# mpsops/mps-bitsandbytes

Measured on AMD Instinct MI355X. Metric: effective bf16 TFLOPS, NF4 dequant+matmul 4096x4096 @ M=4096 (dequantise-once + dense GEMM, two launches), higher is better.
Workload: dtype bf16

## Files before the change

mps_bitsandbytes_amd/csrc/gemm_dense.h:

```cpp
#pragma once
#include "gemm256.h"
#include <type_traits>
#include <utility>

namespace mbnb {

template <int... I, class F> __device__ __forceinline__ void gd_static_for_impl(std::integer_sequence<int, I...>, F &&f) {
    (f(std::integral_constant<int, I>{}), ...);
}
template <int N, class F> __device__ __forceinline__ void gd_static_for(F &&f) {
    gd_static_for_impl(std::make_integer_sequence<int, N>{}, static_cast<F &&>(f));
}

constexpr int GD_LDS = 4 * P_IMG;

template <int FM, int FN = 8> struct GdPlan {
    static_assert(FN == 8 || (FM == 8 && FN >= 5 && FN <= 7), "narrow tiles exist for the 256-row tile only");
    static constexpr int NS = 2 * FN * FM, NR = FN + FM, NP = FN + FM;
    static constexpr int RS1 = (FM == 8 && FN >= 7) ? 2 : 1;
    static constexpr int B1 = FM != 8 ? 16 : (FN == 8 ? 36 : FN == 7 ? 32 : FN == 6 ? 16 : 13), D0 = B1;
    static constexpr int DS = FM == 8 ? 4 : 2;
    static constexpr int B2 = FM != 8 ? 42 : (FN == 8 ? 100 : FN == 7 ? 94 : FN == 6 ? 78 : 66), R0 = B2;
    static_assert(R0 >= FN * FM, "the next tile's slice 0 replaces this tile's only after its MFMAs");
    static_assert((NR - 1) * RS1 < B1, "slice 1 is in registers before barrier 1");
    static_assert(D0 + NP * DS <= B2, "every piece is issued before the vmcnt of barrier 2");
    static_assert(R0 + NR <= NS, "the next tile's slice 0 is in registers before the k-step ends");
};

__device__ __forceinline__ int gd_xcd_major(int bid, int nwg) {
    const int full = (nwg >> 8) << 8;
    if (bid < full) {
        const int i = bid >> 3;
        return (((i >> 5) << 3) + (bid & 7)) * 32 + (i & 31);
    }
    const int rest = nwg - full, r = bid - full, q = rest >> 3, rr = rest & 7, xcd = r & 7;
    return full + (xcd < rr ? xcd * (q + 1) : rr * (q + 1) + (xcd - rr) * q) + (r >> 3);
}
template <int PM, int PN> __device__ __forceinline__ void gd_patch_walk(int v, int tiles_m, int tiles_n, int &tm, int &tn) {
    const int col_tiles = tiles_m * PN, pcs = tiles_n / PN, prs = tiles_m / PM;
    int pc = v / col_tiles, w = PN;
    if (pc >= pcs) { pc = pcs; w = tiles_n - pcs * PN; }
    const int v1 = v - pc * col_tiles;
    int pr = v1 / (PM * w), h = PM;
    if (pr >= prs) { pr = prs; h = tiles_m - prs * PM; }
    const int v2 = v1 - pr * PM * w;
    tm = pr * PM + v2 % h;
    tn = pc * PN + v2 / h;
}

template <typename T, bool SPLITK, int FM, bool I8, int OUTL, int NCH, int FN>
__device__ __forceinline__ void gemm_dense_body(const T *__restrict__ X, const T *__restrict__ Wd, const T *__restrict__ bias,
                                                void *__restrict__ out_v, int out_dtype, float *__restrict__ partial,
                                                int64_t M, int64_t N, int64_t K, int64_t ldw, int64_t k_per_slice,
                                                const float *__restrict__ sA, const float *__restrict__ sB, const OutlierEpilogue &ep,
                                                const int64_t m0, const int64_t n0, const int slice) {
    static_assert(!(I8 && SPLITK), "the int8 form is not split");
    static_assert(OUTL == 0 || I8, "the outlier epilogue belongs to the int8 form");
    static_assert(OUTL == 0 || FN == 8, "the outlier epilogue is written for the 256-wide tile");
    using Frag = typename Mfma16<T>::frag;
    using Plan = GdPlan<FM, FN>;
    constexpr int TM = 32 * FM, TN = 32 * FN;
    extern __shared__ __attribute__((aligned(1024))) char smem[];
    const int tid = threadIdx.x;
    const int lane = tid & 63;
    const int wave = __builtin_amdgcn_readfirstlane(tid >> 6);
    const int wn = wave >> 1, wm = wave & 1;
    const int64_t k_begin = SPLITK ? (int64_t)slice * k_per_slice : 0;
    const int64_t k_len = SPLITK ? (K - k_begin < k_per_slice ? K - k_begin : k_per_slice) : K;
    const int nk = (int)(k_len >> 6);

    typedef int i32x4_t __attribute__((ext_vector_type(4)));
    i32x4_t rs_a, rs_b;
    {
        const uint64_t pa = reinterpret_cast<uint64_t>(X + m0 * K + k_begin), pb = reinterpret_cast<uint64_t>(Wd + n0 * ldw + k_begin);
        const int64_t rows_a = M - m0 < TM ? M - m0 : TM, rows_b = N - n0 < TN ? N - n0 : TN;
        rs_a = i32x4_t{(int)(uint32_t)pa, (int)(uint32_t)(pa >> 32), (int)(rows_a * K * 2), 0x00020000};
        rs_b = i32x4_t{(int)(uint32_t)pb, (int)(uint32_t)(pb >> 32), (int)(rows_b * ldw * 2), 0x00020000};
    }
    int voff_a[FM], voff_b[FN];
#pragma unroll
    for (int pl = 0; pl < FN; pl++) {
        const int row = 8 * (FN * wave + pl) + (lane >> 3);
        voff_b[pl] = (int)(row * ldw * 2) + 16 * ((lane & 7) ^ ((row >> 1) & 7));
    }
#pragma unroll
    for (int pl = 0; pl < FM; pl++) {
        const int row = 8 * (FM * wave + pl) + (lane >> 3);
        voff_a[pl] = (int)(row * K * 2) + 16 * ((lane & 7) ^ ((row >> 1) & 7));
    }
#pragma unroll
    for (int pl = 0; pl < FN; pl++) voff_b[pl] -= (pl & 3) * 1024;
#pragma unroll
    for (int pl = 0; pl < FM; pl++) voff_a[pl] -= (pl & 3) * 1024;
    const uint32_t smem_base = (uint32_t)(uintptr_t)(__attribute__((address_space(3))) void *)smem;
    struct DmaCtx { i32x4_t ra, rb; uint32_t lwa, lwb; };
    auto dma_ctx = [&]() {
        DmaCtx c;
#pragma unroll
        for (int e = 0; e < 4; e++) {
            c.ra[e] = __builtin_amdgcn_readfirstlane(rs_a[e]);
            c.rb[e] = __builtin_amdgcn_readfirstlane(rs_b[e]);
        }
        c.lwa = (uint32_t)__builtin_amdgcn_readfirstlane((int)(smem_base + (uint32_t)(P_A + wave * FM * 1024)));
        c.lwb = (uint32_t)__builtin_amdgcn_readfirstlane((int)(smem_base + (uint32_t)(P_B + wave * FN * 1024)));
        return c;
    };
    auto issue_piece = [&](auto qq, int stage, int kb, const DmaCtx &c) {
        constexpr int q = decltype(qq)::value, pl = q < FM ? q : q - FM;
        const uint32_t dst = (q < FM ? c.lwa : c.lwb) + (uint32_t)(stage * P_IMG + pl * 1024);
        const int vo = (q < FM) ? voff_a[pl] : voff_b[pl];
        const i32x4_t rs = (q < FM) ? c.ra : c.rb;
        if constexpr ((pl & 3) != 0) {
            asm volatile("buffer_load_dwordx4 %0, %1, %2 offen offset:%3 lds" ::"v"(vo), "s"(rs), "s"(kb), "n"((pl & 3) * 1024) : "memory", "m0");
        } else {
            asm volatile("s_mov_b32 m0, %0\n\ts_nop 0\n\tbuffer_load_dwordx4 %1, %2, %3 offen lds" ::"s"(dst), "v"(vo), "s"(rs), "s"(kb) : "memory", "m0");
        }
    };

    const int r16 = lane & 15, fq = lane >> 4;
    int fw[2], fx[2];
#pragma unroll
    for (int ks = 0; ks < 2; ks++) {
        const int f = r16 * ROW_BYTES + (((4 * ks + fq) ^ (r16 >> 1)) << 4);
        fw[ks] = P_B + wn * 16 * FN * ROW_BYTES + f;
        fx[ks] = P_A + wm * 16 * FM * ROW_BYTES + f;
    }
    Frag wf[2][FN], xf[2][FM];
    auto read_one = [&](int stage, auto kk, auto nn) {
        constexpr int ks = decltype(kk)::value, n = decltype(nn)::value;
        if constexpr (n == 0) wf[ks][0] = *reinterpret_cast<const Frag *>(smem + fw[ks] + stage * P_IMG);
        else if constexpr (n <= FM) xf[ks][n - 1] = *reinterpret_cast<const Frag *>(smem + fx[ks] + stage * P_IMG + (n - 1) * 16 * ROW_BYTES);
        else wf[ks][n - FM] = *reinterpret_cast<const Frag *>(smem + fw[ks] + stage * P_IMG + (n - FM) * 16 * ROW_BYTES);
    };
    f32x4 acc[FN][FM];

    auto kbytes = [&](int t) { return t << 7; };

    {
        const DmaCtx c0 = dma_ctx();
        gd_static_for<Plan::NP>([&](auto q) { issue_piece(q, 0, 0, c0); });
        if (nk > 1) {
            gd_static_for<Plan::NP>([&](auto q) { issue_piece(q, 1, kbytes(1), c0); });
            asm volatile("s_waitcnt vmcnt(%0)" ::"n"(Plan::NP) : "memory");
        } else {
            asm volatile("s_waitcnt vmcnt(0)" ::: "memory");
        }
    }
    __builtin_amdgcn_s_barrier();
    asm volatile("" ::: "memory");
    gd_static_for<Plan::NR>([&](auto n) { read_one(0, std::integral_constant<int, 0>{}, n); });

    auto mfma_acc = [&](f32x4 &c, const Frag &a, const Frag &b) {
        if constexpr (I8) asm volatile("v_mfma_i32_16x16x64_i8 %0, %1, %2, %0" : "+a"(c) : "v"(a), "v"(b));
        else if constexpr (std::is_same_v<T, bf16_t>) asm volatile("v_mfma_f32_16x16x32_bf16 %0, %1, %2, %0" : "+a"(c) : "v"(a), "v"(b));
        else asm volatile("v_mfma_f32_16x16x32_f16 %0, %1, %2, %0" : "+a"(c) : "v"(a), "v"(b));
    };
    auto mfma_zero = [&](f32x4 &c, const Frag &a, const Frag &b) {
        if constexpr (I8) asm volatile("v_mfma_i32_16x16x64_i8 %0, %1, %2, 0" : "=a"(c) : "v"(a), "v"(b));
        else if constexpr (std::is_same_v<T, bf16_t>) asm volatile("v_mfma_f32_16x16x32_bf16 %0, %1, %2, 0" : "=a"(c) : "v"(a), "v"(b));
        else asm volatile("v_mfma_f32_16x16x32_f16 %0, %1, %2, 0" : "=a"(c) : "v"(a), "v"(b));
    };

    auto kstep = [&](auto cc, auto first, auto mode_, auto wo_, int j, const DmaCtx &dc) {
        constexpr int WO = decltype(wo_)::value, MODE = decltype(mode_)::value;
        constexpr bool FIRST = decltype(first)::value;
        const int C = cc, Nn = C ^ 1;
        int kb2 = 0;
        if constexpr (MODE == 0) kb2 = __builtin_amdgcn_readfirstlane(kbytes(j + 2));
        gd_static_for<Plan::NS>([&](auto tt) {
            constexpr int t = decltype(tt)::value, ks = t / (FN * FM), f = (t % (FN * FM)) / FM, g = t % FM;
            if constexpr (t == Plan::B1 && MODE != 2) {
                asm volatile("s_waitcnt lgkmcnt(0)" ::: "memory");
                __builtin_amdgcn_s_barrier();
                asm volatile("" ::: "memory");
            }
            if constexpr (t == Plan::B2 && MODE != 2) {
                asm volatile("s_waitcnt vmcnt(%0)" ::"n"(MODE == 0 ? Plan::NP : 0) : "memory");
                __builtin_amdgcn_s_barrier();
                asm volatile("" ::: "memory");
            }
            if constexpr (FIRST && ks == 0) mfma_zero(acc[f][g], wf[ks][f], xf[ks][g]);
            else mfma_acc(acc[f][g], wf[ks][f], xf[ks][g]);
            if constexpr ((t % Plan::RS1) == 0 && t / Plan::RS1 < Plan::NR)
                read_one(C, std::integral_constant<int, 1>{}, std::integral_constant<int, (t / Plan::RS1) % Plan::NR>{});
            if constexpr (MODE != 2 && t >= Plan::R0 && t < Plan::R0 + Plan::NR)
                read_one(Nn, std::integral_constant<int, 0>{}, std::integral_constant<int, (t - Plan::R0) % Plan::NR>{});
            if constexpr (MODE == 0 && t >= Plan::D0 && t < Plan::D0 + Plan::NP * Plan::DS && ((t - Plan::D0) % Plan::DS) == WO)
                issue_piece(std::integral_constant<int, ((t - Plan::D0) / Plan::DS) % Plan::NP>{}, C, kb2, dc);
            __builtin_amdgcn_sched_barrier(0);
        });
    };
    using Mode0 = std::integral_constant<int, 0>;
    using Mode1 = std::integral_constant<int, 1>;
    using Mode2 = std::integral_constant<int, 2>;
    auto main_loop = [&](auto wo) {
        if (nk < 3) return;
        const DmaCtx dc = dma_ctx();
        kstep(std::integral_constant<int, 0>{}, std::true_type{}, Mode0{}, wo, 0, dc);
        int j = 1;
        for (; j + 3 < nk; j += 2) {
            kstep(std::integral_constant<int, 1>{}, std::false_type{}, Mode0{}, wo, j, dc);
            kstep(std::integral_constant<int, 0>{}, std::false_type{}, Mode0{}, wo, j + 1, dc);
        }
        if (j + 2 < nk) kstep(std::integral_constant<int, 1>{}, std::false_type{}, Mode0{}, wo, j, dc);
    };
    if constexpr (Plan::DS == 4) {
        if (wave == 0) main_loop(std::integral_constant<int, 0>{});
        else if (wave == 1) main_loop(std::integral_constant<int, 1>{});
        else if (wave == 2) main_loop(std::integral_constant<int, 2>{});
        else main_loop(std::integral_constant<int, 3>{});
    } else {
        if ((wave & 1) == 0) main_loop(std::integral_constant<int, 0>{});
        else main_loop(std::integral_constant<int, 1>{});
    }

    constexpr bool TAIL = !SPLITK && !I8 && OUTL == 0 && FN == 8;
    bool tail_ok = false;
    if constexpr (TAIL)
        tail_ok = nk >= 2 && out_dtype == (std::is_same_v<T, f16_t> ? MBNB_F16 : MBNB_BF16) && (N % 8 == 0) &&
                  ((reinterpret_cast<uintptr_t>(out_v) & 15) == 0) && N < ((int64_t)1 << 23);
    u32x2 bias_t[TAIL ? FN : 1];
    if constexpr (TAIL) {
        if (tail_ok && bias != nullptr) {
            const uint16_t *bp = reinterpret_cast<const uint16_t *>(bias);
#pragma unroll
            for (int f = 0; f < FN; f++) {
                const int64_t n = n0 + wn * 16 * FN + 16 * f + 4 * fq;
                if (n + 4 <= N && (reinterpret_cast<uintptr_t>(bp + n) & 7) == 0) bias_t[f] = *reinterpret_cast<const u32x2 *>(bp + n);
                else {
                    uint32_t t[4];
#pragma unroll
                    for (int e = 0; e < 4; e++) t[e] = bp[n + e < N ? n + e : N - 1];
                    bias_t[f] = u32x2{t[0] | (t[1] << 16), t[2] | (t[3] << 16)};
                }
            }
        }
    }
    {
        const DmaCtx none{};
        if (nk == 2) kstep(std::integral_constant<int, 0>{}, std::true_type{}, Mode1{}, std::integral_constant<int, 0>{}, 0, none);
        else if (nk > 2) kstep(nk & 1, std::false_type{}, Mode1{}, std::integral_constant<int, 0>{}, nk - 2, none);
        if (nk == 1) kstep(std::integral_constant<int, 0>{}, std::true_type{}, Mode2{}, std::integral_constant<int, 0>{}, 0, none);
        else if (!tail_ok) kstep((nk - 1) & 1, std::false_type{}, Mode2{}, std::integral_constant<int, 0>{}, nk - 1, none);
    }
    if constexpr (TAIL) {
        auto tail_step = [&](auto wb_t, const int C) {
            constexpr bool WB = decltype(wb_t)::value;
            constexpr int ROWB = 264, GS = 2 * FN;
            int tid2 = threadIdx.x;
            asm volatile("" : "+v"(tid2));
            const int lane_e = tid2 & 63, er16 = lane_e & 15, efq = lane_e >> 4;
            char *stg = smem + (wn ? P_B : P_A) + (C ^ 1) * P_IMG + wm * (2 * 16 * ROWB);
            char *st_w = stg + er16 * ROWB + 8 * efq;
            const char *st_r = stg + efq * ROWB + er16 * 16;
            const int64_t m_w = m0 + wm * 16 * FM;
            int64_t rows = M - m_w;
            rows = rows < 0 ? 0 : (rows > 16 * FM ? 16 * FM : rows);
            const uint64_t po = reinterpret_cast<uint64_t>(static_cast<uint16_t *>(out_v) + m_w * N);
            i32x4_t rs_o;
            rs_o[0] = __builtin_amdgcn_readfirstlane((int)(uint32_t)po);
            rs_o[1] = __builtin_amdgcn_readfirstlane((int)(uint32_t)(po >> 32));
            rs_o[2] = __builtin_amdgcn_readfirstlane((int)(rows * N * 2));
            rs_o[3] = 0x00020000;
            const int rowstep = __builtin_amdgcn_readfirstlane((int)(N * 2));
            const int64_t n = n0 + wn * 16 * FN + er16 * 8;
            const int voff0 = n < N ? (int)((efq * N + n) * 2) : (int)0x80000000;
            u32x4 piece[4];
            auto filler = [&](auto gg, auto ss) {
                constexpr int g = decltype(gg)::value, s = decltype(ss)::value, buf = (g & 1) * 16 * ROWB;
                if constexpr (s < FN) {
                    float bv[4] = {0.0f, 0.0f, 0.0f, 0.0f};
                    if constexpr (WB) {
#pragma unroll
                        for (int e = 0; e < 4; e++) bv[e] = unpack_lo<T>(bias_t[s][e >> 1] >> (16 * (e & 1)));
                    }
                    float v[4];
#pragma unroll
                    for (int e = 0; e < 4; e++) {
                        float sv;
                        asm volatile("v_accvgpr_read_b32 %0, %1" : "=v"(sv) : "a"(acc[s][g][e]));
                        v[e] = sv + bv[e];
                    }
                    const u32x2 pk = u32x2{pack2<T>(v[0], v[1]), pack2<T>(v[2], v[3])};
                    *reinterpret_cast<u32x2 *>(st_w + buf + 32 * s) = pk;
                } else if constexpr (s < FN + 4) {
                    constexpr int p = s - FN;
                    const char *srcp = st_r + buf + p * 4 * ROWB;
                    const u32x2 lo = *reinterpret_cast<const u32x2 *>(srcp), hi = *reinterpret_cast<const u32x2 *>(srcp + 8);
                    piece[p] = u32x4{lo[0], lo[1], hi[0], hi[1]};
                } else if constexpr (s < FN + 8) {
                    constexpr int p = s - FN - 4;
                    const int vo = voff0 + (16 * g + 4 * p) * rowstep;
                    const i32x4_t rs = rs_o;
                    const u32x4 pv = piece[p];
                    asm volatile("buffer_store_dwordx4 %0, %1, %2, 0 offen sc1\n\ts_nop 1" ::"v"(pv), "v"(vo), "s"(rs) : "memory");
                }
            };
            gd_static_for<Plan::NS>([&](auto tt) {
                constexpr int t = decltype(tt)::value, g = t / GS, ks = (t % GS) / FN, f = t % FN;
                if constexpr (std::is_same_v<T, bf16_t>) asm volatile("s_nop 1\n\tv_mfma_f32_16x16x32_bf16 %0, %1, %2, %0" : "+a"(acc[f][g]) : "v"(wf[ks][f]), "v"(xf[ks][g]));
                else asm volatile("s_nop 1\n\tv_mfma_f32_16x16x32_f16 %0, %1, %2, %0" : "+a"(acc[f][g]) : "v"(wf[ks][f]), "v"(xf[ks][g]));
                if constexpr (t < Plan::NR)
                    read_one(C, std::integral_constant<int, 1>{},
                             std::integral_constant<int, (t == 0 ? 1 : t == 1 ? 0 : t <= FN ? t - 1 + FM : t - FN + 1)>{});
                if constexpr (t >= GS) filler(std::integral_constant<int, t / GS - 1>{}, std::integral_constant<int, t % GS>{});
                __builtin_amdgcn_sched_barrier(0);
            });
            gd_static_for<GS>([&](auto ss) {
                filler(std::integral_constant<int, FM - 1>{}, ss);
                __builtin_amdgcn_sched_barrier(0);
            });
        };
        if (tail_ok) {
            if (bias != nullptr) tail_step(std::true_type{}, (nk - 1) & 1);
            else tail_step(std::false_type{}, (nk - 1) & 1);
            return;
        }
    }

    asm volatile("s_waitcnt lgkmcnt(0)" ::: "memory");
    __builtin_amdgcn_s_barrier();
    asm volatile("" ::: "memory");
    int tid2 = threadIdx.x;
    asm volatile("" : "+v"(tid2));
    const int lane_e = tid2 & 63, er16 = lane_e & 15, efq = lane_e >> 4;
    const int64_t n_base = n0 + wn * 16 * FN;
    if constexpr (SPLITK) {
        float *o = partial + (int64_t)slice * M * N;
#pragma unroll
        for (int f = 0; f < FN; f++)
#pragma unroll
            for (int g = 0; g < FM; g++) {
                const int64_t m = m0 + wm * 16 * FM + 16 * g + er16, nn = n_base + 16 * f + 4 * efq;
                float v[4];
#pragma unroll
                for (int e = 0; e < 4; e++) asm volatile("v_accvgpr_read_b32 %0, %1" : "=v"(v[e]) : "a"(acc[f][g][e]));
                if (m < M && nn < N) store4_partial(o + m * N + nn, v, nn, N);
                __builtin_amdgcn_sched_barrier(0);
            }
        return;
    }
    if (out_dtype == MBNB_F32) {
        float *o = static_cast<float *>(out_v);
#pragma unroll
        for (int f = 0; f < FN; f++)
#pragma unroll
            for (int g = 0; g < FM; g++) {
                const int64_t m = m0 + wm * 16 * FM + 16 * g + er16, nn = n_base + 16 * f + 4 * efq;
                float v[4];
#pragma unroll
                for (int e = 0; e < 4; e++) {
                    float sv;
                    asm volatile("v_accvgpr_read_b32 %0, %1" : "=v"(sv) : "a"(acc[f][g][e]));
                    if constexpr (I8) {
                        v[e] = (float)__builtin_bit_cast(int, sv) * (sA[m < M ? m : M - 1] / 127.0f) * (sB[nn + e < N ? nn + e : N - 1] / 127.0f);
                    } else {
                        if (bias != nullptr && nn + e < N) sv += to_f32(bias[nn + e]);
                        v[e] = to_f32(from_f32<T>(sv));
                    }
                }
                if (m < M && nn < N) store4(o + m * N + nn, v, nn, N);
                __builtin_amdgcn_sched_barrier(0);
            }
        return;
    }
    constexpr int ROWB = 264;
    char *wave_lds = smem + wave * 64 * ROWB;
    uint16_t *out = static_cast<uint16_t *>(out_v);
    const bool vec_ok = (N % 8 == 0) && ((reinterpret_cast<uintptr_t>(out_v) & 15) == 0);
    const bool same_out = !I8 && out_dtype == (std::is_same_v<T, f16_t> ? MBNB_F16 : MBNB_BF16);
    const bool with_outl = OUTL != 0 && ep.x != nullptr && ep.n_out > 0;
    const bool ow_vec = OUTL != 0 && (ep.n_out % 8 == 0) && ((reinterpret_cast<uintptr_t>(ep.ow) & 15) == 0);
    using OutlT = std::conditional_t<OUTL == 1, f16_t, bf16_t>;
    auto rne = [&](float x) { return to_f32(from_f32<OutlT>(x)); };
    u32x4 wfr_all[OUTL ? 8 * NCH : 1];
    u32x2 bias_all[(OUTL || !I8) ? FN : 1];
    u32x4 xfr_all[OUTL ? FM * NCH : 1];
    if constexpr (!I8) {
        if (bias != nullptr) {
            const uint16_t *bp = reinterpret_cast<const uint16_t *>(bias);
#pragma unroll
            for (int f = 0; f < FN; f++) {
                const int64_t n = n_base + 16 * f + 4 * efq;
                if (n + 4 <= N && (reinterpret_cast<uintptr_t>(bp + n) & 7) == 0) bias_all[f] = *reinterpret_cast<const u32x2 *>(bp + n);
                else {
                    uint32_t t[4];
#pragma unroll
                    for (int e = 0; e < 4; e++) t[e] = bp[n + e < N ? n + e : N - 1];
// ... 109 lines not shown
                    if constexpr (I8) v[e] = (float)__builtin_bit_cast(int, sv) * sa[g] * bv[e];
                    else v[e] = sv + bv[e];
                }
                if constexpr (!I8) {
                    if (!same_out) {
#pragma unroll
                        for (int e = 0; e < 4; e++) v[e] = to_f32(from_f32<T>(v[e]));
                    }
                }
                if constexpr (OUTL != 0) {
                    if constexpr (WO) {
                        f32x4 o = f32x4{0.0f, 0.0f, 0.0f, 0.0f};
                        using OFrag = typename Mfma16<OutlT>::frag;
#pragma unroll
                        for (int c = 0; c < NCH; c++)
                            o = Mfma16<OutlT>::run(__builtin_bit_cast(OFrag, wfr_all[8 * c + f]), __builtin_bit_cast(OFrag, xfr_all[FM * c + GP * H + g]), o);
#pragma unroll
                        for (int e = 0; e < 4; e++) v[e] = rne(rne(v[e]) + rne(o[e]));
                    }
                    if constexpr (WB) {
#pragma unroll
                        for (int e = 0; e < 4; e++) v[e] = rne((WO ? v[e] : rne(v[e])) + bb[e]);
                    }
                }
                u32x2 pk;
                if constexpr (OUTL != 0) pk = u32x2{pack2<OutlT>(v[0], v[1]), pack2<OutlT>(v[2], v[3])};
                else if (out_dtype == MBNB_F16) pk = u32x2{pack2<f16_t>(v[0], v[1]), pack2<f16_t>(v[2], v[3])};
                else pk = u32x2{pack2<bf16_t>(v[0], v[1]), pack2<bf16_t>(v[2], v[3])};
                *reinterpret_cast<u32x2 *>(wave_lds + (16 * g + er16) * ROWB + nl * 2) = pk;
            }
        }
        const int ch = lane_e & 15;
        u32x4 piece[4 * GP];
#pragma unroll
        for (int p = 0; p < 4 * GP; p++) {
            const char *srcp = wave_lds + (p * 4 + (lane_e >> 4)) * ROWB + ch * 16;
            const u32x2 lo = *reinterpret_cast<const u32x2 *>(srcp), hi = *reinterpret_cast<const u32x2 *>(srcp + 8);
            piece[p] = u32x4{lo[0], lo[1], hi[0], hi[1]};
        }
        const int64_t n = n_base + ch * 8;
        if (n < N && ch < 2 * FN) {
            if (vec_ok && n + 8 <= N) {
#pragma unroll
                for (int p = 0; p < 4 * GP; p++) {
                    const int64_t m = m_base + p * 4 + (lane_e >> 4);
                    if (m < M) store_out16(reinterpret_cast<u32x4 *>(out + m * N + n), piece[p]);
                }
            } else {
#pragma unroll
                for (int p = 0; p < 4 * GP; p++) {
                    const int64_t m = m_base + p * 4 + (lane_e >> 4);
                    if (m >= M) continue;
#pragma unroll
                    for (int e = 0; e < 8; e++)
                        if (n + e < N) out[m * N + n + e] = (uint16_t)(piece[p][e >> 1] >> (16 * (e & 1)));
                }
            }
        }
        asm volatile("s_waitcnt lgkmcnt(0)" ::: "memory");
    });
    };
    using Yes = std::true_type;
    using No = std::false_type;
    if constexpr (OUTL != 0) {
        if (with_outl) {
            if (ep.bias != nullptr) epilogue16(Yes{}, Yes{});
            else epilogue16(Yes{}, No{});
        } else {
            if (ep.bias != nullptr) epilogue16(No{}, Yes{});
            else epilogue16(No{}, No{});
        }
    } else if constexpr (!I8) {
        if (bias != nullptr) epilogue16(No{}, Yes{});
        else epilogue16(No{}, No{});
    } else {
        epilogue16(No{}, No{});
    }
}

template <typename T, bool SPLITK, int FM = 8, bool I8 = false, int OUTL = 0, int NCH = 1>
__global__ __launch_bounds__(256, 1) void k_gemm_dense(const T *__restrict__ X, const T *__restrict__ Wd, const T *__restrict__ bias,
                                                       void *__restrict__ out_v, int out_dtype, float *__restrict__ partial,
                                                       int64_t M, int64_t N, int64_t K, int64_t ldw, int64_t k_per_slice,
                                                       const float *__restrict__ sA, const float *__restrict__ sB, OutlierEpilogue ep) {
    constexpr int TM = 32 * FM;
    constexpr int PM = FM == 8 ? 4 : 8, PN = 32 / PM;
    const int tiles_m = (int)((M + TM - 1) / TM), tiles_n = (int)((N + 255) >> 8);
    const int nwg = tiles_m * tiles_n;
    int bid = blockIdx.x, slice = 0;
    if constexpr (SPLITK) {
        slice = bid / nwg;
        bid -= slice * nwg;
    }
    int tm, tn;
    gd_patch_walk<PM, PN>(gd_xcd_major(bid, nwg), tiles_m, tiles_n, tm, tn);
    gemm_dense_body<T, SPLITK, FM, I8, OUTL, NCH, 8>(X, Wd, bias, out_v, out_dtype, partial, M, N, K, ldw, k_per_slice, sA, sB, ep,
                                                     (int64_t)tm * TM, (int64_t)tn << 8, slice);
}

template <typename T, int FNA, int FNB>
__global__ __launch_bounds__(256, 1) void k_gemm_dense_nb(const T *__restrict__ X, const T *__restrict__ Wd, const T *__restrict__ bias,
                                                          void *__restrict__ out_v, int out_dtype, int64_t M, int64_t N, int64_t K,
                                                          int64_t ldw, int tiles_n, int cols_a) {
    const int tiles_m = (int)((M + 255) >> 8);
    int tm, tn;
    gd_patch_walk<4, 8>(gd_xcd_major(blockIdx.x, tiles_m * tiles_n), tiles_m, tiles_n, tm, tn);
    const OutlierEpilogue ep{};
    if (FNA == FNB || tn < cols_a)
        gemm_dense_body<T, false, 8, false, 0, 1, FNA>(X, Wd, bias, out_v, out_dtype, nullptr, M, N, K, ldw, K, nullptr, nullptr, ep,
                                                       (int64_t)tm << 8, (int64_t)tn * (32 * FNA), 0);
    else
        gemm_dense_body<T, false, 8, false, 0, 1, FNB>(X, Wd, bias, out_v, out_dtype, nullptr, M, N, K, ldw, K, nullptr, nullptr, ep,
                                                       (int64_t)tm << 8, (int64_t)cols_a * (32 * FNA) + (int64_t)(tn - cols_a) * (32 * FNB), 0);
}

}
```

mps_bitsandbytes_amd/csrc/gemm_dense.hip:

```cpp
#include <cstdio>
#include "dispatch.h"
#include "gemm_dense.h"
#include "gemm_dense128.h"
#include "gemm_mid.h"

namespace mbnb {

struct DensePlan { int fm; int64_t slices; };
DensePlan gemm_dense_plan(int64_t M, int64_t N, int64_t K) {
    const int64_t tn = (N + 255) / 256, tiles8 = ((M + 255) / 256) * tn, tiles4 = ((M + 127) / 128) * tn;
    const int64_t tiles2 = ((M + 127) / 128) * ((N + 127) / 128);
    const int64_t steps = K / 64;
    DensePlan best{8, 1};
    double best_t = 1e30;
    if (K >= 192 && tiles8 < 96) {
        const int64_t rounds = (tiles2 + 255) / 256;
        best_t = (double)rounds * (double)steps * (tiles2 <= 128 ? 0.36 : 0.47);
        best = DensePlan{2, 1};
    }
    for (int fm = 8; fm >= 4; fm -= 4) {
        const int64_t tiles = fm == 8 ? tiles8 : tiles4;
        const double step = fm == 8 ? 1.3 : 0.75;
        for (int64_t s = 1; s <= 8; s++) {
            const int64_t per = (steps + s - 1) / s;
            if (s > 1 && (per < 8 || tiles8 >= 96)) break;
            const int64_t rounds = (tiles * s + 255) / 256;
            const double t = (double)rounds * (double)per * step + (s > 1 ? 6.0 + 8.0 * (double)s * (double)M * (double)N / 6.0e6 : 0.0);
            if (t < best_t * (fm == 8 ? 1.0 : 0.97)) {
                best_t = t;
                best = DensePlan{fm, s};
            }
        }
    }
    return best;
}
int64_t gemm_dense_slices(int64_t M, int64_t N, int64_t K) { return gemm_dense_plan(M, N, K).slices; }

struct NbPlan { int fna; int cols_a, cols_b; double t_us; };
static double nb_tile_cost(int fn, int64_t nk) {
    static const double fixed[4] = {6.5, 7.0, 7.5, 7.9}, step[4] = {0.85, 1.008, 1.18, 1.30};
    return fixed[fn - 5] + (double)nk * step[fn - 5];
}
static double nb_makespan(int64_t na, double ca, int64_t nb, double cb) {
    const int64_t P = 256, qa = na / P, ra = na % P;
    double lo = (double)qa * ca, hi = lo + ca;
    const int64_t n_lo = P - ra, n_hi = ra;
    double end = na == 0 ? 0.0 : (ra ? hi : lo);
    while (nb > 0) {
        const bool use_lo = n_hi == 0 || lo <= hi;
        const int64_t cap = use_lo ? n_lo : n_hi;
        double &t = use_lo ? lo : hi;
        t += cb;
        if (t > end) end = t;
        nb -= nb < cap ? nb : cap;
    }
    return end;
}
NbPlan gemm_dense_nb_plan(int64_t M, int64_t N, int64_t K, int fm = 8) {
    const int64_t tiles_m = (M + 255) / 256, U = (N + 31) / 32, nk = K / 64;
    const int64_t c8 = (U + 7) / 8, tiles8 = tiles_m * c8;
    const double f = (double)(tiles8 % 256) / 256.0, cost8 = nb_tile_cost(8, nk);
    double uniform_t = cost8 * ((double)(tiles8 / 256) + (f > 0.0 ? (0.3 + 0.7 * f > 0.66 ? 0.3 + 0.7 * f : 0.66) : 0.0));
    if (fm == 4) {
        const int64_t tiles4 = ((M + 127) / 128) * c8;
        uniform_t = (double)((tiles4 + 255) / 256) * (5.0 + 0.75 * (double)nk);
    }
    NbPlan best{8, (int)c8, 0, uniform_t};
    if (tiles8 <= 256 || f == 0.0 || tiles_m > 256 || c8 > (1 << 20)) return best;
    const int64_t span = 256 / tiles_m + 1;
    for (int fna = 8; fna >= 6; fna--) {
        const int fnb = fna - 1;
        const int64_t cmin = (U + fna - 1) / fna, cmax = (U + fnb - 1) / fnb;
        for (int64_t C = cmin; C <= cmax && C <= cmin + span; C++) {
            int64_t a = U - fnb * C;
            if (a < 0) a = 0;
            if (a > C) continue;
            const double t = nb_makespan(tiles_m * a, nb_tile_cost(fna, nk), tiles_m * (C - a), nb_tile_cost(fnb, nk)) * ((a > 0 && a < C) ? 1.02 : 1.0);
            if (t < best.t_us) best = NbPlan{fna, (int)a, (int)(C - a), t};
        }
    }
    if (best.t_us > 0.96 * uniform_t) return NbPlan{8, (int)c8, 0, uniform_t};
    return best;
}
int64_t gemm_dense_k_per_slice(int64_t K, int64_t slices) {
    const int64_t steps = K / 64;
    return ((steps + slices - 1) / slices) * 64;
}
bool gemm_dense_shape(int64_t M, int64_t N, int64_t K, int64_t K_weight) {
    if (K % 64 != 0 || K < 128 || K_weight % 8 != 0) return false;
    if (256 * (K > K_weight ? K : K_weight) * 2 >= ((int64_t)1 << 31)) return false;
    if (M * N * 4 >= ((int64_t)1 << 40)) return false;
    return (M >= 256 && M * N >= 1500000) || (M > 256 && M * N >= 1000000);
}
int64_t gemm_dense_wd_bytes(int64_t N, int64_t K_weight) { return (N * K_weight * 2 + 255) & ~(int64_t)255; }
int64_t gemm_dense_workspace_bytes(int64_t M, int64_t N, int64_t K, int64_t K_weight) {
    if (!gemm_dense_shape(M, N, K, K_weight)) return 0;
    const int64_t s = gemm_dense_slices(M, N, K);
    return gemm_dense_wd_bytes(N, K_weight) + (s > 1 ? s * M * N * 4 : 0);
}

template <typename T, int FM>
static int launch_gemm_dense_fm(const T *x, const T *wd, const T *bias, void *out, int out_dtype, int64_t M, int64_t N, int64_t K,
                                int64_t ldw, float *partial, int64_t slices, hipStream_t st) {
    const int64_t tiles = ((M + 32 * FM - 1) / (32 * FM)) * ((N + 255) / 256);
    if (slices <= 1) {
        auto kern = k_gemm_dense<T, false, FM>;
        if (int rc = ensure_dyn_lds(reinterpret_cast<const void *>(kern), GD_LDS, "matmul_4bit(dense)")) return rc;
        hipLaunchKernelGGL(kern, dim3((unsigned)tiles), dim3(256), GD_LDS, st, x, wd, bias, out, out_dtype, static_cast<float *>(nullptr),
                           M, N, K, ldw, K, static_cast<const float *>(nullptr), static_cast<const float *>(nullptr), OutlierEpilogue{});
        set_kernel_variant("%s", FM == 8 ? "dense 256x256" : "dense 256x128");
        set_kernel_name(FM == 8 ? "dense 256x256" : "dense 256x128");
        return check_launch("matmul_4bit(dense)");
    }
    auto kern = k_gemm_dense<T, true, FM>;
    if (int rc = ensure_dyn_lds(reinterpret_cast<const void *>(kern), GD_LDS, "matmul_4bit(dense split-K)")) return rc;
    const int64_t kps = gemm_dense_k_per_slice(K, slices);
    const int64_t used = (K + kps - 1) / kps;
    hipLaunchKernelGGL(kern, dim3((unsigned)(tiles * used)), dim3(256), GD_LDS, st, x, wd, bias, out, out_dtype, partial, M, N, K, ldw,
                       kps, static_cast<const float *>(nullptr), static_cast<const float *>(nullptr), OutlierEpilogue{});
    if (int rc = check_launch("matmul_4bit(dense split-K)")) return rc;
    const int64_t groups = M * ((N + 3) / 4);
    const unsigned blocks = (unsigned)((groups + 255) / 256);
    if (out_dtype == MBNB_F32)
        hipLaunchKernelGGL((k_splitk_reduce_rm<T, float>), dim3(blocks), dim3(256), 0, st, partial, (int)used, bias, static_cast<float *>(out), M, N);
    else if (out_dtype == MBNB_F16)
        hipLaunchKernelGGL((k_splitk_reduce_rm<T, f16_t>), dim3(blocks), dim3(256), 0, st, partial, (int)used, bias, static_cast<f16_t *>(out), M, N);
    else
        hipLaunchKernelGGL((k_splitk_reduce_rm<T, bf16_t>), dim3(blocks), dim3(256), 0, st, partial, (int)used, bias, static_cast<bf16_t *>(out), M, N);
    set_kernel_variant("%s x%d", FM == 8 ? "dense 256x256" : "dense 256x128", (int)used);
    set_kernel_name(FM == 8 ? "dense 256x256_splitk" : "dense 256x128_splitk");
    return check_launch("matmul_4bit(dense split-K reduce)");
}

template <typename T>
static int launch_gemm_dense_nb(const T *x, const T *wd, const T *bias, void *out, int out_dtype, int64_t M, int64_t N, int64_t K,
                                int64_t ldw, const NbPlan &pl, hipStream_t st) {
    const int tiles_n = pl.cols_a + pl.cols_b;
    const int64_t tiles = ((M + 255) / 256) * tiles_n;
#define MBNB_NB(FNA, FNB)                                                                                                        \
    do {                                                                                                                         \
        auto kern = k_gemm_dense_nb<T, FNA, FNB>;                                                                                \
        if (int rc = ensure_dyn_lds(reinterpret_cast<const void *>(kern), GD_LDS, "matmul_4bit(dense nb)")) return rc;           \
        hipLaunchKernelGGL(kern, dim3((unsigned)tiles), dim3(256), GD_LDS, st, x, wd, bias, out, out_dtype, M, N, K, ldw, tiles_n, \
                           pl.cols_a);                                                                                           \
        set_kernel_variant("dense_nb %d/%d", FNA, FNB);                                                                          \
    } while (0)
    if (pl.fna == 8) MBNB_NB(8, 7);
    else if (pl.fna == 7) MBNB_NB(7, 6);
    else MBNB_NB(6, 5);
#undef MBNB_NB
    static thread_local char name[64];
    snprintf(name, sizeof(name), "dense_nb %dx%d+%dx%d", pl.cols_a, 32 * pl.fna, pl.cols_b, 32 * (pl.fna - 1));
    set_kernel_name(name);
    return check_launch("matmul_4bit(dense nb)");
}

template <typename T>
static int launch_gemm_dense128(const T *x, const T *wd, const T *bias, void *out, int out_dtype, int64_t M, int64_t N, int64_t K,
                                int64_t ldw, hipStream_t st) {
    const int64_t tiles = ((M + 127) / 128) * ((N + 127) / 128);
    auto kern = k_gemm_dense128<T>;
    if (int rc = ensure_dyn_lds(reinterpret_cast<const void *>(kern), G128_LDS, "matmul_4bit(dense128)")) return rc;
    hipLaunchKernelGGL(kern, dim3((unsigned)tiles), dim3(256), G128_LDS, st, x, wd, bias, out, out_dtype, M, N, K, ldw);
    set_kernel_variant("dense 128x128");
    set_kernel_name("dense 128x128");
    return check_launch("matmul_4bit(dense128)");
}

template <typename T>
static int launch_gemm_dense(const T *x, const T *wd, const T *bias, void *out, int out_dtype, int64_t M, int64_t N, int64_t K,
                             int64_t ldw, float *partial, int64_t slices, int fm, hipStream_t st) {
    if (fm == 2) return launch_gemm_dense128<T>(x, wd, bias, out, out_dtype, M, N, K, ldw, st);
    if ((fm == 8 || fm == 4) && slices <= 1) {
        const NbPlan pl = gemm_dense_nb_plan(M, N, K, fm);
        if (pl.cols_b > 0 || pl.fna != 8) return launch_gemm_dense_nb<T>(x, wd, bias, out, out_dtype, M, N, K, ldw, pl, st);
    }
    if (fm == 4 || fm == 10) return launch_gemm_dense_fm<T, 4>(x, wd, bias, out, out_dtype, M, N, K, ldw, partial, slices, st);
    return launch_gemm_dense_fm<T, 8>(x, wd, bias, out, out_dtype, M, N, K, ldw, partial, slices, st);
}

int matmul_4bit_dense_path(const void *A, int64_t M, int64_t K, const uint8_t *packed, const AbsmaxView &am, int64_t N,
                           int64_t K_weight, int blocksize, int qt, int w_dtype, const void *bias, int out_dtype, void *out,
                           void *ws, int64_t ws_bytes, hipStream_t st) {
    if (w_dtype != MBNB_F16 && w_dtype != MBNB_BF16) return MBNB_NOT_APPLICABLE;
    if (!gemm_dense_shape(M, N, K, K_weight) || ws == nullptr) return MBNB_NOT_APPLICABLE;
    if ((reinterpret_cast<uintptr_t>(A) & 15) || (reinterpret_cast<uintptr_t>(ws) & 255) || (reinterpret_cast<uintptr_t>(packed) & 3)) return MBNB_NOT_APPLICABLE;
    const int64_t wd_bytes = gemm_dense_wd_bytes(N, K_weight);
    if (ws_bytes < wd_bytes) return MBNB_NOT_APPLICABLE;
    DensePlan plan = gemm_dense_plan(M, N, K);
    if (plan.slices > 1 && ws_bytes < wd_bytes + plan.slices * M * N * 4) plan.slices = 1;
    const int64_t slices = plan.slices;
    char *wsb = static_cast<char *>(ws);
    if (int rc = dequantize_4bit_dispatch(packed, am, N, K_weight, K_weight, blocksize, qt, w_dtype, wsb, st, N * K_weight <= (int64_t(1) << 25) ? 2 : (M >= 2048 ? 1 : 0))) return rc;
    float *partial = reinterpret_cast<float *>(wsb + wd_bytes);
    int rc;
    if (w_dtype == MBNB_F16)
        rc = launch_gemm_dense<f16_t>(static_cast<const f16_t *>(A), reinterpret_cast<const f16_t *>(wsb), static_cast<const f16_t *>(bias),
                                      out, out_dtype, M, N, K, K_weight, partial, slices, plan.fm, st);
    else
        rc = launch_gemm_dense<bf16_t>(static_cast<const bf16_t *>(A), reinterpret_cast<const bf16_t *>(wsb),
                                       static_cast<const bf16_t *>(bias), out, out_dtype, M, N, K, K_weight, partial, slices, plan.fm, st);
    set_kernel_name(slices > 1 ? "dequant+dense_splitk" : "dequant+dense");
    return rc;
}

int linear8_dense_path(const void *X, int dtype, int64_t M, int64_t K, const void *W, const float *scales, int64_t N, bool fp8,
                       const void *bias, void *out, void *ws, int64_t ws_bytes, hipStream_t st) {
    if (dtype != MBNB_F16 && dtype != MBNB_BF16) return MBNB_NOT_APPLICABLE;
    if (!gemm_dense_shape(M, N, K, K) || ws == nullptr) return MBNB_NOT_APPLICABLE;
    if ((reinterpret_cast<uintptr_t>(X) & 15) || (reinterpret_cast<uintptr_t>(ws) & 255)) return MBNB_NOT_APPLICABLE;
    const int64_t wd_bytes = gemm_dense_wd_bytes(N, K);
    if (ws_bytes < wd_bytes) return MBNB_NOT_APPLICABLE;
    DensePlan plan = gemm_dense_plan(M, N, K);
    if (plan.slices > 1 && ws_bytes < wd_bytes + plan.slices * M * N * 4) plan.slices = 1;
    const int64_t slices = plan.slices;
    char *wsb = static_cast<char *>(ws);
    const int policy = N * K <= (int64_t(1) << 25) ? 2 : (M >= 2048 ? 1 : 0);
    const int rcq = fp8 ? dequantize_fp8_dispatch(static_cast<const uint8_t *>(W), scales, N, K, dtype, wsb, st, policy)
                        : dequantize_rowwise_dispatch(static_cast<const int8_t *>(W), scales, N, K, dtype, wsb, st, policy);
    if (rcq) return rcq;
    float *partial = reinterpret_cast<float *>(wsb + wd_bytes);
    int rc;
    if (dtype == MBNB_F16)
        rc = launch_gemm_dense<f16_t>(static_cast<const f16_t *>(X), reinterpret_cast<const f16_t *>(wsb), static_cast<const f16_t *>(bias),
                                      out, dtype, M, N, K, K, partial, slices, plan.fm, st);
    else
        rc = launch_gemm_dense<bf16_t>(static_cast<const bf16_t *>(X), reinterpret_cast<const bf16_t *>(wsb),
                                       static_cast<const bf16_t *>(bias), out, dtype, M, N, K, K, partial, slices, plan.fm, st);
    set_kernel_name(fp8 ? (slices > 1 ? "fp8a16_dequant+dense_splitk" : "fp8a16_dequant+dense")
                        : (slices > 1 ? "w8a16_dequant+dense_splitk" : "w8a16_dequant+dense"));
    return rc;
}

bool gemm_i8_dense_shape(int64_t M, int64_t N, int64_t K) {
    return (K % 128 == 0) && K >= 256 && 256 * K < ((int64_t)1 << 31) && ((M + 255) / 256) * ((N + 255) / 256) >= 96;
}
bool gemm_i8_dense_outlier_ok(const OutlierEpilogue &ep, int out_dtype) {
    return out_dtype != MBNB_F32 && (ep.x == nullptr || ep.n_out == 0 || (ep.ldx <= 64 && ep.ldx % 16 == 0 && (reinterpret_cast<uintptr_t>(ep.x) & 15) == 0));
}
int launch_gemm_i8_dense(const int8_t *A, const int8_t *Bt, const float *sA, const float *sB, int64_t M, int64_t N, int64_t K,
                         int out_dtype, void *out, hipStream_t st, const OutlierEpilogue *ep) {
    const int64_t tiles = ((M + 255) / 256) * ((N + 255) / 256);
    if (ep != nullptr) {
        const bool two = ep->x != nullptr && ep->n_out > 0 && ep->ldx > 32;
        auto kern = out_dtype == MBNB_F16 ? (two ? k_gemm_dense<bf16_t, false, 8, true, 1, 2> : k_gemm_dense<bf16_t, false, 8, true, 1, 1>)
                                          : (two ? k_gemm_dense<bf16_t, false, 8, true, 2, 2> : k_gemm_dense<bf16_t, false, 8, true, 2, 1>);
        if (int rc = ensure_dyn_lds(reinterpret_cast<const void *>(kern), GD_LDS, "matmul_int8(dense+outliers)")) return rc;
        hipLaunchKernelGGL(kern, dim3((unsigned)tiles), dim3(256), GD_LDS, st, reinterpret_cast<const bf16_t *>(A),
                           reinterpret_cast<const bf16_t *>(Bt), static_cast<const bf16_t *>(nullptr), out, out_dtype,
                           static_cast<float *>(nullptr), M, N, K / 2, K / 2, K / 2, sA, sB, *ep);
        set_kernel_variant("i8_dense OUTL%d NCH%d", out_dtype == MBNB_F16 ? 1 : 2, two ? 2 : 1);
        return check_launch("matmul_int8(dense+outliers)");
    }
    auto kern = k_gemm_dense<bf16_t, false, 8, true>;
    if (int rc = ensure_dyn_lds(reinterpret_cast<const void *>(kern), GD_LDS, "matmul_int8(dense)")) return rc;
    hipLaunchKernelGGL(kern, dim3((unsigned)tiles), dim3(256), GD_LDS, st, reinterpret_cast<const bf16_t *>(A),
                       reinterpret_cast<const bf16_t *>(Bt), static_cast<const bf16_t *>(nullptr), out, out_dtype,
                       static_cast<float *>(nullptr), M, N, K / 2, K / 2, K / 2, sA, sB, OutlierEpilogue{});
    set_kernel_variant("i8_dense");
    return check_launch("matmul_int8(dense)");
}

int gemm_dense_direct(const void *A, const void *Wd, int dtype, const void *bias, int out_dtype, void *out, int64_t M, int64_t N,
                      int64_t K, int64_t ldw, float *partial, int64_t slices, int tile_m, int forced_cols_a, hipStream_t st) {
    if (tile_m >= 640) {
        const int fnb = tile_m / 128, fna = fnb + 1;
        const int64_t U = (N + 31) / 32;
        int64_t a = forced_cols_a;
        if (a * fna > U) a = U / fna;
        const int64_t b = (U - a * fna + fnb - 1) / fnb;
        const NbPlan pl{fna, (int)a, (int)b, 0.0};
        if (dtype == MBNB_F16)
            return launch_gemm_dense_nb<f16_t>(static_cast<const f16_t *>(A), static_cast<const f16_t *>(Wd), static_cast<const f16_t *>(bias), out, out_dtype, M, N, K, ldw, pl, st);
        return launch_gemm_dense_nb<bf16_t>(static_cast<const bf16_t *>(A), static_cast<const bf16_t *>(Wd), static_cast<const bf16_t *>(bias), out, out_dtype, M, N, K, ldw, pl, st);
    }
    const int fm = tile_m == 128 ? 10 : (tile_m == 256 ? 9 : (tile_m == 384 ? 2 : gemm_dense_plan(M, N, K).fm));
    if (dtype == MBNB_F16)
        return launch_gemm_dense<f16_t>(static_cast<const f16_t *>(A), static_cast<const f16_t *>(Wd), static_cast<const f16_t *>(bias), out,
                                        out_dtype, M, N, K, ldw, partial, slices, fm, st);
    return launch_gemm_dense<bf16_t>(static_cast<const bf16_t *>(A), static_cast<const bf16_t *>(Wd), static_cast<const bf16_t *>(bias), out,
                                     out_dtype, M, N, K, ldw, partial, slices, fm, st);
}

}
```

Before: 1375.

## Precompute tile-walk reciprocal, hoist M0 writes, pipeline accumulator reads in epilogue

The host now computes a fixed-point reciprocal, so the kernel's patch-walk tile mapping can replace its integer division with a multiply-high when the tile counts divide the patch evenly. In the main loop, the M0 register setup for each group-leading LDS DMA piece moves one step earlier, which removes the s_nop before that buffer_load. In the epilogue, accumulators are read out of AGPRs a couple of steps ahead into VGPR buffers. The final k-step MFMAs then accumulate in VGPRs without the s_nop padding, overlapping the AGPR reads with compute. This raises VGPR pressure and makes the hazard timing around M0 and MFMA more delicate.

```diff
diff --git a/mps_bitsandbytes_amd/csrc/gemm_dense.h b/mps_bitsandbytes_amd/csrc/gemm_dense.h
--- a/mps_bitsandbytes_amd/csrc/gemm_dense.h
+++ b/mps_bitsandbytes_amd/csrc/gemm_dense.h
@@ -27,7 +27,7 @@
     static_assert(R0 + NR <= NS, "the next tile's slice 0 is in registers before the k-step ends");
 };
 
-__device__ __forceinline__ int gd_xcd_major(int bid, int nwg) {
+__host__ __device__ __forceinline__ int gd_xcd_major(int bid, int nwg) {
     const int full = (nwg >> 8) << 8;
     if (bid < full) {
         const int i = bid >> 3;
@@ -36,7 +36,22 @@
     const int rest = nwg - full, r = bid - full, q = rest >> 3, rr = rest & 7, xcd = r & 7;
     return full + (xcd < rr ? xcd * (q + 1) : rr * (q + 1) + (xcd - rr) * q) + (r >> 3);
 }
-template <int PM, int PN> __device__ __forceinline__ void gd_patch_walk(int v, int tiles_m, int tiles_n, int &tm, int &tn) {
+template <int PM, int PN> __host__ __device__ __forceinline__ uint32_t gd_walk_rcp(int64_t tiles_m, int64_t tiles_n) {
+    const int64_t d = tiles_m * PN;
+    if (tiles_m <= 0 || tiles_n <= 0 || tiles_m % PM != 0 || tiles_n % PN != 0 || tiles_m * tiles_n * d >= ((int64_t)1 << 32)) return 0u;
+    return (uint32_t)((((int64_t)1 << 32) / d) + 1);
+}
+template <int PM, int PN>
+__host__ __device__ __forceinline__ void gd_patch_walk(int v, int tiles_m, int tiles_n, int &tm, int &tn, uint32_t col_rcp = 0u) {
+    static_assert((PM & (PM - 1)) == 0 && (PN & (PN - 1)) == 0, "the whole-patch path divides by PM and PM * PN with shifts");
+    if (col_rcp != 0u) {
+        const int pc = (int)(uint32_t)(((uint64_t)(uint32_t)v * col_rcp) >> 32);
+        const unsigned v1 = (unsigned)(v - pc * (tiles_m * PN));
+        const unsigned pr = v1 / (unsigned)(PM * PN), v2 = v1 % (unsigned)(PM * PN);
+        tm = (int)(pr * PM + v2 % (unsigned)PM);
+        tn = pc * PN + (int)(v2 / (unsigned)PM);
+        return;
+    }
     const int col_tiles = tiles_m * PN, pcs = tiles_n / PN, prs = tiles_m / PM;
     int pc = v / col_tiles, w = PN;
     if (pc >= pcs) { pc = pcs; w = tiles_n - pcs * PN; }
@@ -105,12 +120,20 @@
         c.lwb = (uint32_t)__builtin_amdgcn_readfirstlane((int)(smem_base + (uint32_t)(P_B + wave * FN * 1024)));
         return c;
     };
-    auto issue_piece = [&](auto qq, int stage, int kb, const DmaCtx &c) {
+    auto piece_m0 = [&](auto qq, int stage, const DmaCtx &c) {
+        constexpr int q = decltype(qq)::value, pl = q < FM ? q : q - FM;
+        static_assert((pl & 3) == 0, "pieces 4 g .. 4 g + 3 share the M0 of piece 4 g");
+        const uint32_t dst = (q < FM ? c.lwa : c.lwb) + (uint32_t)(stage * P_IMG + pl * 1024);
+        asm volatile("s_mov_b32 m0, %0" ::"s"(dst) : "memory", "m0");
+    };
+    auto issue_piece = [&](auto qq, auto m0_ahead, int stage, int kb, const DmaCtx &c) {
         constexpr int q = decltype(qq)::value, pl = q < FM ? q : q - FM;
         const uint32_t dst = (q < FM ? c.lwa : c.lwb) + (uint32_t)(stage * P_IMG + pl * 1024);
         const int vo = (q < FM) ? voff_a[pl] : voff_b[pl];
         const i32x4_t rs = (q < FM) ? c.ra : c.rb;
-        if constexpr ((pl & 3) != 0) {
+        if constexpr ((pl & 3) == 0 && decltype(m0_ahead)::value) {
+            asm volatile("buffer_load_dwordx4 %0, %1, %2 offen lds" ::"v"(vo), "s"(rs), "s"(kb) : "memory", "m0");
+        } else if constexpr ((pl & 3) != 0) {
             asm volatile("buffer_load_dwordx4 %0, %1, %2 offen offset:%3 lds" ::"v"(vo), "s"(rs), "s"(kb), "n"((pl & 3) * 1024) : "memory", "m0");
         } else {
             asm volatile("s_mov_b32 m0, %0\n\ts_nop 0\n\tbuffer_load_dwordx4 %1, %2, %3 offen lds" ::"s"(dst), "v"(vo), "s"(rs), "s"(kb) : "memory", "m0");
@@ -138,9 +161,9 @@
 
     {
         const DmaCtx c0 = dma_ctx();
-        gd_static_for<Plan::NP>([&](auto q) { issue_piece(q, 0, 0, c0); });
+        gd_static_for<Plan::NP>([&](auto q) { issue_piece(q, std::false_type{}, 0, 0, c0); });
         if (nk > 1) {
-            gd_static_for<Plan::NP>([&](auto q) { issue_piece(q, 1, kbytes(1), c0); });
+            gd_static_for<Plan::NP>([&](auto q) { issue_piece(q, std::false_type{}, 1, kbytes(1), c0); });
             asm volatile("s_waitcnt vmcnt(%0)" ::"n"(Plan::NP) : "memory");
         } else {
             asm volatile("s_waitcnt vmcnt(0)" ::: "memory");
@@ -186,7 +209,11 @@
             if constexpr (MODE != 2 && t >= Plan::R0 && t < Plan::R0 + Plan::NR)
                 read_one(Nn, std::integral_constant<int, 0>{}, std::integral_constant<int, (t - Plan::R0) % Plan::NR>{});
             if constexpr (MODE == 0 && t >= Plan::D0 && t < Plan::D0 + Plan::NP * Plan::DS && ((t - Plan::D0) % Plan::DS) == WO)
-                issue_piece(std::integral_constant<int, ((t - Plan::D0) / Plan::DS) % Plan::NP>{}, C, kb2, dc);
+                issue_piece(std::integral_constant<int, ((t - Plan::D0) / Plan::DS) % Plan::NP>{}, std::true_type{}, C, kb2, dc);
+            if constexpr (MODE == 0 && t + 1 >= Plan::D0 && t + 1 < Plan::D0 + Plan::NP * Plan::DS && ((t + 1 - Plan::D0) % Plan::DS) == WO) {
+                constexpr int qn = ((t + 1 - Plan::D0) / Plan::DS) % Plan::NP;
+                if constexpr ((((qn < FM) ? qn : qn - FM) & 3) == 0) piece_m0(std::integral_constant<int, qn>{}, C, dc);
+            }
             __builtin_amdgcn_sched_barrier(0);
         });
     };
@@ -266,20 +293,26 @@
             const int64_t n = n0 + wn * 16 * FN + er16 * 8;
             const int voff0 = n < N ? (int)((efq * N + n) * 2) : (int)0x80000000;
             u32x4 piece[4];
+            f32x4 cv[2][FN];
+            auto fetch = [&](auto gg, auto ff) {
+                constexpr int g = decltype(gg)::value, f = decltype(ff)::value;
+#pragma unroll
+                for (int e = 0; e < 4; e++) {
+                    float sv;
+                    const f32x4 &av = acc[f][g];
+                    asm volatile("v_accvgpr_read_b32 %0, %1" : "=v"(sv) : "a"(av[e]));
+                    f32x4 &cc = cv[g & 1][f];
+                    cc[e] = sv;
+                }
+            };
             auto filler = [&](auto gg, auto ss) {
                 constexpr int g = decltype(gg)::value, s = decltype(ss)::value, buf = (g & 1) * 16 * ROWB;
                 if constexpr (s < FN) {
-                    float bv[4] = {0.0f, 0.0f, 0.0f, 0.0f};
-                    if constexpr (WB) {
-#pragma unroll
-                        for (int e = 0; e < 4; e++) bv[e] = unpack_lo<T>(bias_t[s][e >> 1] >> (16 * (e & 1)));
-                    }
                     float v[4];
 #pragma unroll
                     for (int e = 0; e < 4; e++) {
-                        float sv;
-                        asm volatile("v_accvgpr_read_b32 %0, %1" : "=v"(sv) : "a"(acc[s][g][e]));
-                        v[e] = sv + bv[e];
+                        v[e] = cv[g & 1][s][e];
+                        if constexpr (WB) v[e] += unpack_lo<T>(bias_t[s][e >> 1] >> (16 * (e & 1)));
                     }
                     const u32x2 pk = u32x2{pack2<T>(v[0], v[1]), pack2<T>(v[2], v[3])};
                     *reinterpret_cast<u32x2 *>(st_w + buf + 32 * s) = pk;
@@ -296,14 +329,18 @@
                     asm volatile("buffer_store_dwordx4 %0, %1, %2, 0 offen sc1\n\ts_nop 1" ::"v"(pv), "v"(vo), "s"(rs) : "memory");
                 }
             };
+            fetch(std::integral_constant<int, 0>{}, std::integral_constant<int, 0>{});
+            fetch(std::integral_constant<int, 0>{}, std::integral_constant<int, 1>{});
+            __builtin_amdgcn_sched_barrier(0);
             gd_static_for<Plan::NS>([&](auto tt) {
                 constexpr int t = decltype(tt)::value, g = t / GS, ks = (t % GS) / FN, f = t % FN;
-                if constexpr (std::is_same_v<T, bf16_t>) asm volatile("s_nop 1\n\tv_mfma_f32_16x16x32_bf16 %0, %1, %2, %0" : "+a"(acc[f][g]) : "v"(wf[ks][f]), "v"(xf[ks][g]));
-                else asm volatile("s_nop 1\n\tv_mfma_f32_16x16x32_f16 %0, %1, %2, %0" : "+a"(acc[f][g]) : "v"(wf[ks][f]), "v"(xf[ks][g]));
+                if constexpr (std::is_same_v<T, bf16_t>) asm volatile("v_mfma_f32_16x16x32_bf16 %0, %1, %2, %0" : "+v"(cv[g & 1][f]) : "v"(wf[ks][f]), "v"(xf[ks][g]));
+                else asm volatile("v_mfma_f32_16x16x32_f16 %0, %1, %2, %0" : "+v"(cv[g & 1][f]) : "v"(wf[ks][f]), "v"(xf[ks][g]));
                 if constexpr (t < Plan::NR)
                     read_one(C, std::integral_constant<int, 1>{},
                              std::integral_constant<int, (t == 0 ? 1 : t == 1 ? 0 : t <= FN ? t - 1 + FM : t - FN + 1)>{});
                 if constexpr (t >= GS) filler(std::integral_constant<int, t / GS - 1>{}, std::integral_constant<int, t % GS>{});
+                if constexpr ((t + 2) % GS < FN && (t + 2) / GS < FM) fetch(std::integral_constant<int, (t + 2) / GS>{}, std::integral_constant<int, (t + 2) % GS>{});
                 __builtin_amdgcn_sched_barrier(0);
             });
             gd_static_for<GS>([&](auto ss) {
@@ -579,7 +616,8 @@
 __global__ __launch_bounds__(256, 1) void k_gemm_dense(const T *__restrict__ X, const T *__restrict__ Wd, const T *__restrict__ bias,
                                                        void *__restrict__ out_v, int out_dtype, float *__restrict__ partial,
                                                        int64_t M, int64_t N, int64_t K, int64_t ldw, int64_t k_per_slice,
-                                                       const float *__restrict__ sA, const float *__restrict__ sB, OutlierEpilogue ep) {
+                                                       const float *__restrict__ sA, const float *__restrict__ sB, OutlierEpilogue ep,
+                                                       uint32_t walk_rcp) {
     constexpr int TM = 32 * FM;
     constexpr int PM = FM == 8 ? 4 : 8, PN = 32 / PM;
     const int tiles_m = (int)((M + TM - 1) / TM), tiles_n = (int)((N + 255) >> 8);
@@ -590,7 +628,7 @@
         bid -= slice * nwg;
     }
     int tm, tn;
-    gd_patch_walk<PM, PN>(gd_xcd_major(bid, nwg), tiles_m, tiles_n, tm, tn);
+    gd_patch_walk<PM, PN>(gd_xcd_major(bid, nwg), tiles_m, tiles_n, tm, tn, walk_rcp);
     gemm_dense_body<T, SPLITK, FM, I8, OUTL, NCH, 8>(X, Wd, bias, out_v, out_dtype, partial, M, N, K, ldw, k_per_slice, sA, sB, ep,
                                                      (int64_t)tm * TM, (int64_t)tn << 8, slice);
 }
@@ -598,10 +636,10 @@
 template <typename T, int FNA, int FNB>
 __global__ __launch_bounds__(256, 1) void k_gemm_dense_nb(const T *__restrict__ X, const T *__restrict__ Wd, const T *__restrict__ bias,
                                                           void *__restrict__ out_v, int out_dtype, int64_t M, int64_t N, int64_t K,
-                                                          int64_t ldw, int tiles_n, int cols_a) {
+                                                          int64_t ldw, int tiles_n, int cols_a, uint32_t walk_rcp) {
     const int tiles_m = (int)((M + 255) >> 8);
     int tm, tn;
-    gd_patch_walk<4, 8>(gd_xcd_major(blockIdx.x, tiles_m * tiles_n), tiles_m, tiles_n, tm, tn);
+    gd_patch_walk<4, 8>(gd_xcd_major(blockIdx.x, tiles_m * tiles_n), tiles_m, tiles_n, tm, tn, walk_rcp);
     const OutlierEpilogue ep{};
     if (FNA == FNB || tn < cols_a)
         gemm_dense_body<T, false, 8, false, 0, 1, FNA>(X, Wd, bias, out_v, out_dtype, nullptr, M, N, K, ldw, K, nullptr, nullptr, ep,
diff --git a/mps_bitsandbytes_amd/csrc/gemm_dense.hip b/mps_bitsandbytes_amd/csrc/gemm_dense.hip
--- a/mps_bitsandbytes_amd/csrc/gemm_dense.hip
+++ b/mps_bitsandbytes_amd/csrc/gemm_dense.hip
@@ -103,11 +103,12 @@
 static int launch_gemm_dense_fm(const T *x, const T *wd, const T *bias, void *out, int out_dtype, int64_t M, int64_t N, int64_t K,
                                 int64_t ldw, float *partial, int64_t slices, hipStream_t st) {
     const int64_t tiles = ((M + 32 * FM - 1) / (32 * FM)) * ((N + 255) / 256);
+    const uint32_t walk_rcp = gd_walk_rcp<(FM == 8 ? 4 : 8), (FM == 8 ? 8 : 4)>((M + 32 * FM - 1) / (32 * FM), (N + 255) / 256);
     if (slices <= 1) {
         auto kern = k_gemm_dense<T, false, FM>;
         if (int rc = ensure_dyn_lds(reinterpret_cast<const void *>(kern), GD_LDS, "matmul_4bit(dense)")) return rc;
         hipLaunchKernelGGL(kern, dim3((unsigned)tiles), dim3(256), GD_LDS, st, x, wd, bias, out, out_dtype, static_cast<float *>(nullptr),
-                           M, N, K, ldw, K, static_cast<const float *>(nullptr), static_cast<const float *>(nullptr), OutlierEpilogue{});
+                           M, N, K, ldw, K, static_cast<const float *>(nullptr), static_cast<const float *>(nullptr), OutlierEpilogue{}, walk_rcp);
         set_kernel_variant("%s", FM == 8 ? "dense 256x256" : "dense 256x128");
         set_kernel_name(FM == 8 ? "dense 256x256" : "dense 256x128");
         return check_launch("matmul_4bit(dense)");
@@ -117,7 +118,7 @@
     const int64_t kps = gemm_dense_k_per_slice(K, slices);
     const int64_t used = (K + kps - 1) / kps;
     hipLaunchKernelGGL(kern, dim3((unsigned)(tiles * used)), dim3(256), GD_LDS, st, x, wd, bias, out, out_dtype, partial, M, N, K, ldw,
-                       kps, static_cast<const float *>(nullptr), static_cast<const float *>(nullptr), OutlierEpilogue{});
+                       kps, static_cast<const float *>(nullptr), static_cast<const float *>(nullptr), OutlierEpilogue{}, walk_rcp);
     if (int rc = check_launch("matmul_4bit(dense split-K)")) return rc;
     const int64_t groups = M * ((N + 3) / 4);
     const unsigned blocks = (unsigned)((groups + 255) / 256);
@@ -142,7 +143,7 @@
         auto kern = k_gemm_dense_nb<T, FNA, FNB>;                                                                                \
         if (int rc = ensure_dyn_lds(reinterpret_cast<const void *>(kern), GD_LDS, "matmul_4bit(dense nb)")) return rc;           \
         hipLaunchKernelGGL(kern, dim3((unsigned)tiles), dim3(256), GD_LDS, st, x, wd, bias, out, out_dtype, M, N, K, ldw, tiles_n, \
-                           pl.cols_a);                                                                                           \
+                           pl.cols_a, gd_walk_rcp<4, 8>((M + 255) / 256, tiles_n));                                              \
         set_kernel_variant("dense_nb %d/%d", FNA, FNB);                                                                          \
     } while (0)
     if (pl.fna == 8) MBNB_NB(8, 7);
@@ -241,6 +242,7 @@
 int launch_gemm_i8_dense(const int8_t *A, const int8_t *Bt, const float *sA, const float *sB, int64_t M, int64_t N, int64_t K,
                          int out_dtype, void *out, hipStream_t st, const OutlierEpilogue *ep) {
     const int64_t tiles = ((M + 255) / 256) * ((N + 255) / 256);
+    const uint32_t walk_rcp = gd_walk_rcp<4, 8>((M + 255) / 256, (N + 255) / 256);
     if (ep != nullptr) {
         const bool two = ep->x != nullptr && ep->n_out > 0 && ep->ldx > 32;
         auto kern = out_dtype == MBNB_F16 ? (two ? k_gemm_dense<bf16_t, false, 8, true, 1, 2> : k_gemm_dense<bf16_t, false, 8, true, 1, 1>)
@@ -248,7 +250,7 @@
         if (int rc = ensure_dyn_lds(reinterpret_cast<const void *>(kern), GD_LDS, "matmul_int8(dense+outliers)")) return rc;
         hipLaunchKernelGGL(kern, dim3((unsigned)tiles), dim3(256), GD_LDS, st, reinterpret_cast<const bf16_t *>(A),
                            reinterpret_cast<const bf16_t *>(Bt), static_cast<const bf16_t *>(nullptr), out, out_dtype,
-                           static_cast<float *>(nullptr), M, N, K / 2, K / 2, K / 2, sA, sB, *ep);
+                           static_cast<float *>(nullptr), M, N, K / 2, K / 2, K / 2, sA, sB, *ep, walk_rcp);
         set_kernel_variant("i8_dense OUTL%d NCH%d", out_dtype == MBNB_F16 ? 1 : 2, two ? 2 : 1);
         return check_launch("matmul_int8(dense+outliers)");
     }
@@ -256,7 +258,7 @@
     if (int rc = ensure_dyn_lds(reinterpret_cast<const void *>(kern), GD_LDS, "matmul_int8(dense)")) return rc;
     hipLaunchKernelGGL(kern, dim3((unsigned)tiles), dim3(256), GD_LDS, st, reinterpret_cast<const bf16_t *>(A),
                        reinterpret_cast<const bf16_t *>(Bt), static_cast<const bf16_t *>(nullptr), out, out_dtype,
-                       static_cast<float *>(nullptr), M, N, K / 2, K / 2, K / 2, sA, sB, OutlierEpilogue{});
+                       static_cast<float *>(nullptr), M, N, K / 2, K / 2, K / 2, sA, sB, OutlierEpilogue{}, walk_rcp);
     set_kernel_variant("i8_dense");
     return check_launch("matmul_int8(dense)");
 }
```

Result: no change. 1386 (median of 6 runs) (+0.8%).
